# sonniki/image-captioning-with-external-knowledge

Hardware: AMD Instinct MI355X
Metric: decode_steps_per_sec (higher is better)
Workload: dtype f32 (3xbf16 split products, fp32 accumulate); 1 GPU; cfg2: geo variant, per-GPU batch 64 x 20 decode positions, 14x14x2048 features, K=20 knowledge rows, vocab 10000; global_batch=64, graph=True, collective_backend=none, split_allreduce=False, parallelism=dp1 (one flat-bucket all-reduce per step)

## Files before the change

### image-captioning-with-external-knowledge_amd/csrc/attention.hip

```cpp
#include <cstdlib>

#include "attention_mfma.h"
#include "common.h"

namespace ick {
namespace {

template <int DHP, bool VEC>
__global__ __launch_bounds__(256) void attn_kernel(ick_attn_args p, int TQ, int SLD) {
    chain_priority();
    constexpr int VLD = DHP + 4;
    constexpr int G = DHP / 4;
    extern __shared__ __attribute__((aligned(16))) float smem[];
    const int S = p.S, dh = p.dh;
    float* Vs = smem;
    float* Qs = Vs + S * VLD;
    float* Ps = Qs + TQ * DHP;
    float* rowinv = Ps + TQ * SLD;

    const int h = blockIdx.x, b = blockIdx.y, t0 = blockIdx.z * TQ;
    const int nt = min(TQ, p.T - t0);
    const int tid = threadIdx.x, lane = tid & 63, wave = tid >> 6;
    const Dropout drop = make_dropout(p.drop_p, epoch_seed(p.drop_seed, p.drop_epoch), p.drop_site);
    int slen = S;
// ... 318 lines not shown
    if (dir == 0) {
        pl.tq = attn_fwd_chunk(T, S, DHP);
        if (attn_fwd_floats(pl.tq, S, DHP) > kAttnBudget) return ICK_EINVAL;
    } else {
        pl.tq = attn_bwd_chunk(T, S, DHP);
        if (attn_bwd_floats(pl.tq, S, DHP) > kAttnBudget) return ICK_EINVAL;
    }
    pl.chunks = ceil_div(T, pl.tq);
    pl.overwrites = dir == 0 || pl.chunks == 1;
    return 0;
}

}
}

extern "C" int ick_attention(const ick_attn_args* in, void* stream) {
    using namespace ick;
    if (!in) return ICK_EINVAL;
    const ick_attn_args& a = *in;
    ICK_CHECK_ARG(a.Q && a.K && a.V && a.O);
    ICK_CHECK_ARG(a.B > 0 && a.H > 0 && a.T > 0 && a.S > 0 && a.dh > 0 && a.dh <= 64);
    ICK_CHECK_ARG(a.B <= 65535);
    hipStream_t s = (hipStream_t)stream;
    AttnPlan pl;
    if (int e = attn_plan(0, a.T, a.S, a.dh, attn_head_major(a, a.dh <= 32 ? 32 : 64), pl)) return e;
    if (pl.mfma) return launch_attn_mfma(a, s);
    if (pl.dhp == 32) return launch_attn<32>(a, pl.tq, s);
    return launch_attn<64>(a, pl.tq, s);
}


extern "C" int ick_attention_bwd(const ick_attn_bwd_args* in, void* stream) {
    using namespace ick;
    if (!in) return ICK_EINVAL;
    const ick_attn_bwd_args& a = *in;
    ICK_CHECK_ARG(a.Q && a.K && a.V && a.O && a.dO && a.lse && a.dQ && a.dK && a.dV);
    ICK_CHECK_ARG(a.B > 0 && a.B <= 65535 && a.H > 0 && a.T > 0 && a.S > 0 && a.dh > 0 && a.dh <= 64);
    const int DHP = a.dh <= 32 ? 32 : 64;
    ICK_CHECK_ARG(attn_head_major(a, DHP));
    hipStream_t s = (hipStream_t)stream;
    AttnPlan pl;
    if (int e = attn_plan(1, a.T, a.S, a.dh, true, pl)) return e;
    if (pl.mfma) return launch_attn_bwd_mfma(a, s);
    if (pl.dhp == 32) return launch_attn_bwd<32>(a, pl.tq, s);
    return launch_attn_bwd<64>(a, pl.tq, s);
}

extern "C" int ick_attention_bwd_overwrites(int32_t T, int32_t S, int32_t dh) {
    using namespace ick;
    AttnPlan pl;
    return attn_plan(1, T, S, dh, true, pl) == 0 && pl.overwrites ? 1 : 0;
}

extern "C" int ick_attention_plan(int32_t dir, int32_t T, int32_t S, int32_t dh, int32_t head_major, int32_t* out) {
    using namespace ick;
    if (!out) return ICK_EINVAL;
    AttnPlan pl;
    const int e = attn_plan(dir, T, S, dh, head_major != 0, pl);
    const int v[7] = {pl.mfma, pl.nqt, pl.maxt, pl.dhp, pl.tq, pl.chunks, pl.overwrites};
    for (int i = 0; i < 7; ++i) out[i] = v[i];
    return e;
}
```

### image-captioning-with-external-knowledge_amd/csrc/attention_mfma.h

```cpp
#pragma once
#include "common.h"

namespace ick {

constexpr int kAttnMfmaUnsupported = -1000;

bool attn_mfma_shape_ok(int T, int S, int dh);
int attn_mfma_nqt(int T);
int attn_mfma_maxt(int S);
template <class Args>
inline bool attn_head_major(const Args& a, int DHP) {
    auto al16 = [](const void* q) { return (reinterpret_cast<uintptr_t>(q) & 15) == 0; };
    return a.q_ts == DHP && a.k_ss == DHP && a.v_ss == DHP && al16(a.Q) && al16(a.K) && al16(a.V) && a.q_bs % 4 == 0 &&
           a.q_hs % 4 == 0 && a.k_bs % 4 == 0 && a.k_hs % 4 == 0 && a.v_bs % 4 == 0 && a.v_hs % 4 == 0;
}
int launch_attn_mfma(const ick_attn_args& a, hipStream_t s);
int launch_attn_bwd_mfma(const ick_attn_bwd_args& a, hipStream_t s);

}
```

### image-captioning-with-external-knowledge_amd/csrc/attention_mfma.hip

```cpp
#include <algorithm>

#include "attention_mfma.h"

#ifdef ICK_ATTN_STAMPS
__device__ unsigned long long ick_attn_stamps[4][16];
#define ICK_ASTAMP(kern, i)                                                                   \
    do {                                                                                      \
        if (threadIdx.x == 0 && blockIdx.x == 0 && blockIdx.y == 0) ick_attn_stamps[kern][i] = __builtin_readcyclecounter(); \
    } while (0)
extern "C" int ick_debug_read_attn_stamps(unsigned long long* out) {
    return (int)hipMemcpyFromSymbol(out, HIP_SYMBOL(ick_attn_stamps), sizeof(ick_attn_stamps));
}
#else
#define ICK_ASTAMP(kern, i)
#endif

namespace ick {
namespace {

constexpr int DHP = 32;
constexpr int QLD = DHP + 4;

__device__ __forceinline__ float4 mask_cols(float4 x, int c0, int dh) {
    x.x = c0 + 0 < dh ? x.x : 0.f; x.y = c0 + 1 < dh ? x.y : 0.f;
    x.z = c0 + 2 < dh ? x.z : 0.f; x.w = c0 + 3 < dh ? x.w : 0.f;
    return x;
}

__device__ __forceinline__ int wave_id_of(unsigned tid) { return __builtin_amdgcn_readfirstlane((int)(tid >> 6)); }

__device__ __forceinline__ f32x4 mfma4(const float4& a, const float4& b, f32x4 c) {
    c = __builtin_amdgcn_mfma_f32_16x16x4f32(a.x, b.x, c, 0, 0, 0);
    c = __builtin_amdgcn_mfma_f32_16x16x4f32(a.y, b.y, c, 0, 0, 0);
    c = __builtin_amdgcn_mfma_f32_16x16x4f32(a.z, b.z, c, 0, 0, 0);
    c = __builtin_amdgcn_mfma_f32_16x16x4f32(a.w, b.w, c, 0, 0, 0);
    return c;
}

template <int IT>
__device__ __forceinline__ void stage_transposed_load(const float* __restrict__ src, int rows, float4 (&x)[IT]) {
#pragma unroll
    for (int it = 0; it < IT; ++it) {
        const int f = threadIdx.x + 256 * it;
        const int s = f >> 3, c = f & 7;
        x[it] = *reinterpret_cast<const float4*>(src + (int64_t)(s < rows ? s : 0) * DHP + 4 * c);
    }
}
template <int IT>
__device__ __forceinline__ void stage_transposed_store(const float4 (&x)[IT], float* __restrict__ dst, int rows,
                                                       int rows_pad, int SP, int dh) {
#pragma unroll
    for (int it = 0; it < IT; ++it) {
        const int f = threadIdx.x + 256 * it;
        const int s = f >> 3, c = f & 7;
        if (s < rows_pad) {
            const float4 v = mask_cols(x[it], 4 * c, s < rows ? dh : 0);
            dst[(4 * c + 0) * SP + s] = v.x; dst[(4 * c + 1) * SP + s] = v.y;
            dst[(4 * c + 2) * SP + s] = v.z; dst[(4 * c + 3) * SP + s] = v.w;
// ... 116 lines not shown
        }
        s += __shfl_xor(s, 16, 64);
        s += __shfl_xor(s, 32, 64);
        sum[qt] = s;
    }
    f32x4 oacc[NQT][2];
#pragma unroll
    for (int qt = 0; qt < NQT; ++qt) {
#pragma unroll
        for (int jt = 0; jt < 2; ++jt) {
            f32x4 acc = {0.f, 0.f, 0.f, 0.f};
#pragma unroll
            for (int i = 0; i < MAXT; ++i) {
                if (wave + 4 * i < nkt) {
                    const float4 vt = *reinterpret_cast<const float4*>(Vt + (16 * jt + li) * SP + 16 * (wave + 4 * i) + 4 * lq);
                    const float4 pf = make_float4(sc[i][qt][0], sc[i][qt][1], sc[i][qt][2], sc[i][qt][3]);
                    acc = mfma4(vt, pf, acc);
                }
            }
            oacc[qt][jt] = acc;
        }
        if (lq == 0) rsum[wave * NQ + 16 * qt + li] = sum[qt];
    }
    ICK_ASTAMP(SK, 6);
    __syncthreads();
    ICK_ASTAMP(SK, 7);
#pragma unroll
    for (int qt = 0; qt < NQT; ++qt)
#pragma unroll
        for (int jt = 0; jt < 2; ++jt)
            *reinterpret_cast<f32x4*>(Ored + ((wave * NQT + qt) * 2 + jt) * 256 + lane * 4) = oacc[qt][jt];
    if (tid < NQ) {
        const float s = (rsum[tid] + rsum[NQ + tid]) + (rsum[2 * NQ + tid] + rsum[3 * NQ + tid]);
        stat[NQ + tid] = s > 0.f ? 1.f / s : 0.f;
        if (p.lse && tid < T) p.lse[((int64_t)b * p.H + h) * T + tid] = stat[tid] + __logf(s);
    }
    __syncthreads();
    for (int tt = wave; tt < NQT * 2; tt += 4) {
        const int qt = tt >> 1, jt = tt & 1;
        f32x4 o = {0.f, 0.f, 0.f, 0.f};
#pragma unroll
        for (int w = 0; w < 4; ++w) o += *reinterpret_cast<const f32x4*>(Ored + ((w * NQT + qt) * 2 + jt) * 256 + lane * 4);
        const int query = 16 * qt + li;
        if (query < T) {
            const float inv = stat[NQ + query];
            float* orow = p.O + (int64_t)b * p.o_bs + (int64_t)query * p.o_ts + h * dh;
            const int j0 = 16 * jt + 4 * lq;
#pragma unroll
            for (int r = 0; r < 4; ++r)
                if (j0 + r < dh) orow[j0 + r] = o[r] * inv;
        }
    }
    ICK_ASTAMP(SK, 8);
}

template <int NQT, int MAXT>
__global__ __launch_bounds__(256) void attn_bwd_mfma_kernel(ick_attn_bwd_args p, int SP, bool st2) {
    chain_priority_bwd();
    [[maybe_unused]] constexpr int SK = MAXT > 1 ? 3 : 2;
    ICK_ASTAMP(SK, 0);
    constexpr int NQ = NQT * 16;
    constexpr int TLD = NQ + 4;
    extern __shared__ __attribute__((aligned(16))) float smem[];
    const int TR = (p.T + 3) & ~3;
    float* dSs = smem;
    float* Qs = dSs + TR * SP;
    float* Gs = Qs + NQ * QLD;
    float* Qt = Gs + NQ * QLD;
    float* Gt = Qt + DHP * TLD;
    float* Ls = Gt + DHP * TLD;
    float* Dl = Ls + NQ;
    float* Kw = Dl + NQ + (wave_id_of(threadIdx.x)) * (16 * QLD);
    float* dQp = Qs;

    const int b = blockIdx.x, h = blockIdx.y;
    const int tid = threadIdx.x, lane = tid & 63, wave = tid >> 6;
    const int li = lane & 15, lq = lane >> 4;
    const int T = p.T, S = p.S, dh = p.dh;
    const int nkt = (S + 15) >> 4;
    const Dropout drop = make_dropout(p.drop_p, epoch_seed(p.drop_seed, p.drop_epoch), p.drop_site);
    const float* qb = p.Q + (int64_t)b * p.q_bs + (int64_t)h * p.q_hs;
    const float* kb = p.K + (int64_t)b * p.k_bs + (int64_t)h * p.k_hs;
    const float* vb = p.V + (int64_t)b * p.v_bs + (int64_t)h * p.v_hs;
    const float* ob = p.O + (int64_t)b * p.o_bs + h * dh;
    const float* gb = p.dO + (int64_t)b * p.o_bs + h * dh;

    constexpr int QIT = (NQ * 8 + 255) / 256;
    float4 qx[QIT];
#pragma unroll
    for (int it = 0; it < QIT; ++it) {
        const int f = tid + 256 * it;
        const int t = f >> 3, c = f & 7;
        qx[it] = *reinterpret_cast<const float4*>(qb + (int64_t)(t < T ? t : 0) * DHP + 4 * c);
    }
    const float lse_v = p.lse[((int64_t)b * p.H + h) * T + (tid < T ? tid : 0)];
    float gv[NQT * 2], ov[NQT * 2];
#pragma unroll
    for (int it = 0; it < NQT * 2; ++it) {
        const int f = tid + 256 * it;
        const int t = f >> 5, j = f & 31;
        const bool ok = t < T && j < dh;
        const int64_t at = ok ? (int64_t)t * p.o_ts + j : 0;
        gv[it] = gb[at];
        ov[it] = ob[at];
    }
    float4 kf[MAXT][2], vf[MAXT][2];
// ... 145 lines not shown
        const int qt = tt >> 1, jt = tt & 1;
        const int j = 16 * jt + li;
        f32x4 acc = {0.f, 0.f, 0.f, 0.f};
#pragma unroll
        for (int w = 0; w < 4; ++w) acc += *reinterpret_cast<const f32x4*>(dQp + ((w * NQT + qt) * 2 + jt) * 256 + lane * 4);
        if (j < dh) {
#pragma unroll
            for (int r = 0; r < 4; ++r) {
                const int query = 16 * qt + 4 * lq + r;
                if (query < T) p.dQ[(int64_t)b * p.dq_bs + (int64_t)query * p.dq_ts + h * dh + j] = acc[r];
            }
        }
    }
    ICK_ASTAMP(SK, 6);
}

template <int NQT, int MAXT>
int launch_fwd(const ick_attn_args& a, int SP, hipStream_t s) {
    const size_t fl = std::max<size_t>((size_t)DHP * SP, 4 * NQT * 2 * 256) + (size_t)NQT * 16 * QLD + 10 * NQT * 16;
    if (fl * sizeof(float) > 150 * 1024) return kAttnMfmaUnsupported;
    auto kern = attn_fwd_mfma_kernel<NQT, MAXT>;
    static LdsAttrOnce attr;
    if (int e = attr.ensure((const void*)kern, 160 * 1024)) return e;
    hipLaunchKernelGGL(kern, dim3(a.H, a.B), dim3(256), fl * sizeof(float), s, a, SP);
    ICK_LAUNCH_RET();
}

template <int NQT, int MAXT>
int launch_bwd(const ick_attn_bwd_args& a, int SP, hipStream_t s) {
    constexpr int NQ = NQT * 16;
    const size_t tr = (size_t)((a.T + 3) & ~3);
    const size_t fl = std::max(tr * SP + 2 * (size_t)NQ * QLD + 2 * (size_t)DHP * (NQ + 4) + 2 * NQ + 4 * 16 * QLD,
                               (size_t)NQ * SP + 64);
    if (fl * sizeof(float) > 150 * 1024) return kAttnMfmaUnsupported;
    auto kern = attn_bwd_mfma_kernel<NQT, MAXT>;
    static LdsAttrOnce attr;
    if (int e = attr.ensure((const void*)kern, 160 * 1024)) return e;
    const bool st2 = a.dh % 2 == 0 && a.dk_bs % 2 == 0 && a.dk_ss % 2 == 0 && a.dv_bs % 2 == 0 && a.dv_ss % 2 == 0 &&
                     (reinterpret_cast<uintptr_t>(a.dK) & 7) == 0 && (reinterpret_cast<uintptr_t>(a.dV) & 7) == 0;
    hipLaunchKernelGGL(kern, dim3(a.B, a.H), dim3(256), fl * sizeof(float), s, a, SP, st2);
    ICK_LAUNCH_RET();
}

}

bool attn_mfma_shape_ok(int T, int S, int dh) {
    if (!(T >= 2 && T <= 64 && S >= 1 && S <= 512 && dh <= DHP)) return false;
    const size_t nq = (size_t)((T + 15) / 16) * 16, sp = (size_t)((S + 15) / 16) * 16 + 4, tr = (size_t)((T + 3) & ~3);
    return std::max(tr * sp + 2 * nq * QLD + 2 * DHP * (nq + 4) + 2 * nq + 4 * 16 * QLD, nq * sp + 64) * sizeof(float) <= 150 * 1024;
}

int attn_mfma_nqt(int T) { return (T + 15) / 16; }

int attn_mfma_maxt(int S) { return S <= 64 ? 1 : (S <= 256 ? 4 : (S <= 320 ? 5 : 8)); }

int launch_attn_mfma(const ick_attn_args& a, hipStream_t s) {
    if (!attn_mfma_shape_ok(a.T, a.S, a.dh)) return kAttnMfmaUnsupported;
    if (!attn_head_major(a, DHP)) return kAttnMfmaUnsupported;
    const int SP = ((a.S + 15) / 16) * 16 + 4;
    const int nqt = attn_mfma_nqt(a.T);
    const int mt = attn_mfma_maxt(a.S);
#define ICK_FWD(N)                                                                                   \
    case N: return mt == 1 ? launch_fwd<N, 1>(a, SP, s) : (mt == 4 ? launch_fwd<N, 4>(a, SP, s) :   \
                   (mt == 5 ? launch_fwd<N, 5>(a, SP, s) : launch_fwd<N, 8>(a, SP, s)))
    switch (nqt) {
        ICK_FWD(1); ICK_FWD(2); ICK_FWD(3); ICK_FWD(4);
    }
#undef ICK_FWD
    return kAttnMfmaUnsupported;
}

int launch_attn_bwd_mfma(const ick_attn_bwd_args& a, hipStream_t s) {
    if (!attn_mfma_shape_ok(a.T, a.S, a.dh)) return kAttnMfmaUnsupported;
    const int SP = ((a.S + 15) / 16) * 16 + 4;
    const int mt = attn_mfma_maxt(a.S);
#define ICK_BWD(N)                                                                                   \
    case N: return mt == 1 ? launch_bwd<N, 1>(a, SP, s) : (mt == 4 ? launch_bwd<N, 4>(a, SP, s) :   \
                   (mt == 5 ? launch_bwd<N, 5>(a, SP, s) : launch_bwd<N, 8>(a, SP, s)))
    switch (attn_mfma_nqt(a.T)) {
        ICK_BWD(1); ICK_BWD(2); ICK_BWD(3); ICK_BWD(4);
    }
#undef ICK_BWD
    return kAttnMfmaUnsupported;
}

}
```

### image-captioning-with-external-knowledge_amd/lib.py

```python
import ctypes as C
import os

_PKG = os.path.dirname(os.path.abspath(__file__))
LIB_PATH = os.path.join(_PKG, "libick_amd.so")
if os.environ.get("ICK_LIB_PATH"):
    LIB_PATH = os.environ["ICK_LIB_PATH"]

ICK_GEO, ICK_KNOWLEDGE, ICK_NEWS = 0, 1, 2
VARIANT_ID = {"geo": ICK_GEO, "knowledge": ICK_KNOWLEDGE, "news": ICK_NEWS}
GEMM_RELU, GEMM_ACCUM, GEMM_ATOMIC, GEMM_COLSUM_ONLY = 1, 2, 4, 16

vp = C.c_void_p
i32 = C.c_int32
i64 = C.c_int64
f32 = C.c_float
u32 = C.c_uint32


class GemmArgs(C.Structure):
    _fields_ = [
        ("A", vp), ("B", vp), ("C", vp), ("bias", vp),
        ("M", i32), ("N", i32), ("K", i32),
        ("a_rs", i64), ("a_ks", i64), ("a_grp", i32), ("a_gs", i64), ("a_gmap", vp),
        ("b_rs", i64), ("b_ks", i64),
# ... 145 lines not shown
    "ick_gemm": [C.POINTER(GemmArgs), vp],
    "ick_gemm_plan": [C.POINTER(GemmArgs), C.POINTER(GemmPlanInfo)],
    "ick_set_gemm_split": [i32],
    "ick_get_gemm_split": [],
    "ick_presplit_bytes": [i32, i32, C.POINTER(i64)],
    "ick_presplit_weights": [C.POINTER(PresplitItem), i32, vp],
    "ick_rowchain_supported": [i32, i32, i32],
    "ick_rowchain_fwd": [C.POINTER(RowChainArgs), vp],
    "ick_rowchain_bwd_supported": [i32, i32, i32],
    "ick_rowchain_bwd": [C.POINTER(RowChainBwdArgs), vp],
    "ick_pack_weights": [C.POINTER(PackItem), i32, vp],
    "ick_packed_weight_floats": [i32, i32, C.POINTER(i64)],
    "ick_add_layernorm": [vp, vp, vp, vp, vp, i64, i32, f32, i64, i64, i64, vp, vp, f32, u32, u32, vp, vp],
    "ick_attention": [C.POINTER(AttnArgs), vp],
    "ick_entity_encode": [i32, vp, i32, vp, vp, i32, vp, i32, vp, i32, i32, i32, i32, vp],
    "ick_fact_encode": [vp, vp, vp, i32, vp, i32, i32, i32, i32, vp],
    "ick_caption_embed": [vp, vp, vp, vp, vp, vp, vp, vp, i32, i32, i32, i32, i32, i32, i32, f32, i32, f32, u32, u32,
                          vp, vp],
    "ick_context_indicators": [vp, vp, vp, vp, vp, vp, i32, i32, i32, i32, i32, i32, i32, i32, i32, vp],
    "ick_pointer_scores": [vp, vp, vp, vp, vp, vp, i32, i32, i32, i32, i64, i32, vp, vp],
    "ick_mul": [vp, vp, vp, i64, vp],
    "ick_dropout_mask": [vp, i64, i32, f32, u32, u32, vp],
    "ick_top2": [vp, i64, i32, i32, vp, vp, vp],
    "ick_greedy_update": [vp, vp, vp, vp, vp, vp, vp, i32, i32, i32, i32, i32, i32, i32, vp],
    "ick_greedy_select": [vp, i64, i32, i32, vp, vp, vp, vp, vp, i32, i32, i32, i32, i32, i32, vp],
    "ick_packed_ce": [vp, i64, vp, vp, i32, i32, i32, i32, vp, vp, vp, vp, vp],
    "ick_packed_ce_weighted": [vp, i64, vp, vp, vp, i32, i32, i32, i32, vp, vp, vp, vp, vp],
    "ick_samples_to_captions": [vp, i32, i32, i32, i32, i32, i32, i32, i32, vp, vp, vp, vp],
    "ick_cider_d": [vp, i32, i32, vp, i32, i32, i32, vp, vp, i32, f32, f32, i32, i32, i32, vp, i32, i32, vp, i32,
                    vp, vp, vp],
    "ick_decode_supported": [i32, i32, i32, i32, i32],
    "ick_decode_plan": [i32, i32, i32, i32, i32, C.POINTER(i32)],
    "ick_decode_layers": [C.POINTER(DecodeCtx), i32, vp],
    "ick_decode_layers_part": [C.POINTER(DecodeCtx), i32, i32, vp],
    "ick_decode_layers_attn": [C.POINTER(DecodeCtx), vp, i32, i32, vp],
    "ick_decode_init": [C.POINTER(DecodeCtx), i32, i32, vp],
    "ick_decode_select_greedy": [C.POINTER(DecodeCtx), i32, vp],
    "ick_decode_select_beam": [C.POINTER(DecodeCtx), C.POINTER(BeamState), i32, vp],
    "ick_decode_beam_supported": [i32, i32],
    "ick_decode_select_sample": [C.POINTER(DecodeCtx), C.POINTER(SampleState), i32, vp],
    "ick_decode_sample_supported": [i32, i32],
    "ick_decode_select_beam_rules": [C.POINTER(DecodeCtx), C.POINTER(BeamState), C.POINTER(DecodeRules), i32, vp],
    "ick_decode_select_sample_rules": [C.POINTER(DecodeCtx), C.POINTER(SampleState), C.POINTER(DecodeRules), i32, vp],
    "ick_decode_select_beam_diverse": [C.POINTER(DecodeCtx), C.POINTER(BeamState), C.POINTER(DecodeRules),
                                       C.POINTER(DecodeDiversity), i32, vp],
    "ick_decode_select_beam_forced": [C.POINTER(DecodeCtx), C.POINTER(BeamState), C.POINTER(DecodeRules),
                                      C.POINTER(DecodeConstraints), i32, vp],
    "ick_attention_bwd": [C.POINTER(AttnBwdArgs), vp],
    "ick_layernorm_bwd": [vp, vp, vp, vp, vp, vp, vp, vp, vp, i64, i32, vp, f32, u32, u32, vp, vp, vp],
    "ick_layernorm_bwd_rows_per_block": [],
    "ick_gemm_grouped": [vp, i32, vp],
    "ick_attention_bwd_overwrites": [i32, i32, i32],
    "ick_attention_plan": [i32, i32, i32, i32, i32, C.POINTER(i32)],
    "ick_relu_bwd": [vp, vp, vp, i64, f32, vp],
    "ick_colsum": [vp, i64, i32, i64, vp, vp],
    "ick_caption_embed_bwd": [vp, vp, vp, vp, vp, vp, i32, i32, i32, i32, i32, i32, i32, f32, f32, u32, u32, vp, vp],
    "ick_pointer_scores_bwd": [vp, i64, i32, vp, vp, vp, vp, vp, vp, vp, vp, i32, i32, i32, i32, vp],
    "ick_entity_encode_bwd": [i32, vp, vp, i32, vp, vp, i32, vp, i32, vp, i32, i32, i32, vp],
    "ick_fact_encode_bwd": [vp, vp, vp, vp, i32, i32, i32, i32, i32, vp],
    "ick_context_gate_bwd": [vp, vp, vp, vp, vp, i32, i32, i32, i32, i32, i32, i32, i32, i32, vp],
    "ick_adam_clamp": [vp, vp, vp, vp, i64, f32, f32, f32, f32, f32, f32, i32, vp, vp, vp],
    "ick_adam_clamp_derive": [vp, vp, vp, vp, vp, vp, i32, f32, f32, f32, f32, f32, f32, i32, vp, vp, vp],
    "ick_grad_sqnorm_plan": [i64, C.POINTER(i32)],
    "ick_grad_sqnorm": [vp, i64, f32, vp, vp, i64, vp, vp],
    "ick_adam_opt": [vp, vp, vp, vp, i64, f32, f32, vp, LrSchedule, f32, f32, f32, i32, vp, vp, vp],
    "ick_adam_opt_derive": [vp, vp, vp, vp, vp, vp, i32, f32, f32, vp, LrSchedule, f32, f32, f32, i32, vp, vp, vp],
    "ick_adam_ema": [vp, vp, vp, vp, vp, i64, f32, f32, f32, vp, LrSchedule, f32, f32, f32, i32, vp, vp, vp, i32, vp],
    "ick_adam_ema_derive": [vp, vp, vp, vp, vp, vp, vp, i32, f32, f32, f32, vp, LrSchedule, f32, f32, f32, i32, vp, vp, vp,
                            i32, vp],
    "ick_adam_decay": [vp, vp, vp, vp, vp, i64, f32, f32, f32, vp, LrSchedule, f32, f32, f32, i32, vp, vp, vp, i32, vp, vp,
                       i64, i32, vp],
    "ick_adam_decay_derive": [vp, vp, vp, vp, vp, vp, vp, i32, f32, f32, f32, vp, LrSchedule, f32, f32, f32, i32, vp, vp, vp,
                              i32, vp, vp, i64, i32, vp],
    "ick_conv1_wgrad_plan": [i32, i32, i32, i32, C.POINTER(i32), C.POINTER(i64)],
    "ick_conv1_wgrad": [vp, vp, vp, vp, i32, i32, i32, i32, vp, i64, vp],
    "ick_counter_add": [vp, u32, vp],
    "ick_counter_add_if": [vp, u32, vp, vp],
    "ick_timestamp": [vp, vp],
    "ick_copy_batch": [vp, vp, vp, i32, vp],
    "ick_scale_by_ratio": [vp, i64, vp, vp, vp],
    "ick_head_rowmap": [vp, i32, i32, vp, vp, vp, vp],
    "ick_pointer_scores_packed": [vp, vp, vp, vp, vp, vp, i32, i32, i32, i32, i64, i32, vp, vp, vp],
    "ick_packed_ce_packed": [vp, i64, vp, vp, vp, vp, i32, i32, i32, i32, vp, vp, vp, vp, vp],
    "ick_packed_ce_smooth": [vp, i64, vp, vp, vp, vp, vp, vp, i32, i32, i32, i32, vp, vp, vp, vp, vp],
    "ick_pointer_scores_bwd_packed": [vp, i64, i32, vp, vp, vp, vp, vp, vp, vp, vp, i32, i32, i32, i32, vp, vp, vp],
    "ick_gather_rows": [vp, i64, vp, vp, vp, i64, i32, i32, vp],
    "ick_row_logprob_rank": [vp, i64, vp, vp, vp, i32, i32, i32, i32, vp, vp, vp, vp],
    "ick_caption_score_sums": [vp, i32, i32, i32, vp, vp, vp, vp, vp, vp, vp, vp, vp, vp],
    "ick_sched_sample_mix": [vp, i64, vp, vp, vp, vp, i32, i32, i32, i32, i32, i32, i32, vp, vp, vp, vp, i32, vp, vp, vp,
                             vp],
    "ick_caption_metrics": [vp, i32, i32, vp, i32, i32, i32, i32, i32, i32, vp, i32, i32, C.c_double, i32, vp, i32, vp,
                            vp, vp, vp, vp, vp, vp, vp, vp],
    "ick_caption_metric_sums": [vp, vp, vp, i32, vp, vp, vp, vp],
    "ick_geo_reference_counts": [vp, i32, i32, vp, vp, vp, i32, i32, i32, i32, C.POINTER(i32), i32, i32, i32, vp, i32, vp,
                                 i32, i32, i64, i64, i64, vp, vp, vp, vp],
}

_lib = None
PROFILE = None
_proxy = None


class IckError(RuntimeError):
    pass


# ... 28 lines not shown
```

### image-captioning-with-external-knowledge_amd/ops.py

```python
import contextlib
import ctypes as C
import gc
import math
import os

import torch

from . import lib as L


def _p(t):
    return None if t is None else t.data_ptr()


def _stream():
    return torch.cuda.current_stream().cuda_stream


def _f32c(t, name):
    if t.dtype != torch.float32 or not t.is_cuda:
        raise L.IckError("%s must be a float32 device tensor (got %s on %s)" % (name, t.dtype, t.device))
    return t


# ... 901 lines not shown
    if N < 1 or not 1 <= T <= GEO_MAX_T:
        raise L.IckError("geo_reference_counts: N >= 1 and 1 <= T <= %d (got %d, %d)" % (GEO_MAX_T, N, T))
    if B < 1 or not 1 <= K <= GEO_MAX_K or Cf < 5:
        raise L.IckError("geo_reference_counts: entities need B >= 1, 1 <= K <= %d and C >= 5" % GEO_MAX_K)
    if tuple(entity_names.shape) != (B, K, 2 + GEO_NAME_CHARS):
        raise L.IckError("geo_reference_counts: entity_names must be (%d, %d, %d)" % (B, K, 2 + GEO_NAME_CHARS))
    for t, name in ((bins_distance, "bins_distance"), (bins_azimuth, "bins_azimuth")):
        if t.shape[1] != 2 or not 1 <= t.shape[0] <= GEO_MAX_BINS:
            raise L.IckError("geo_reference_counts: %s holds 1..%d [lo, hi] rows" % (name, GEO_MAX_BINS))
    if isinstance(n_types, bool) or not isinstance(n_types, int) or not 1 <= n_types <= GEO_MAX_TYPES:
        raise L.IckError("geo_reference_counts: 1 <= n_types <= %d" % GEO_MAX_TYPES)
    trigger_ids = [int(i) for i in trigger_ids]
    ids = trigger_ids + [int(of_id), int(the_id), int(a_id)]
    if len(trigger_ids) != GEO_TERMS or not isinstance(V, int) or V < 1 or not all(-1 <= i < V for i in ids):
        raise L.IckError("geo_reference_counts: 8 trigger ids and the ids of of / the / a, each -1 or in [0, V)")
    if not isinstance(image_index, torch.Tensor) or image_index.shape != (N,):
        raise L.IckError("geo_reference_counts needs an (N,) image_index")
    if not 0 <= int(row_offset) <= 2 ** 62 or not -2 ** 63 <= int(seed) < 2 ** 64:
        raise L.IckError("geo_reference_counts: row_offset >= 0 and a 64-bit seed")
    dev = tokens.device
    idx = image_index.to(device=dev, dtype=torch.int32).contiguous()
    seed = int(seed) & (2 ** 64 - 1)
    seed -= 2 ** 64 if seed >= 2 ** 63 else 0
    ld = 1 + 2 * GEO_MAX_BINS + (n_types + 63) // 64 * 64
    hist = torch.zeros(2, GEO_TERMS, ld, device=dev, dtype=torch.int32)
    marks = torch.empty(N, T, device=dev, dtype=torch.int32)
    trig = (C.c_int32 * GEO_TERMS)(*trigger_ids)
    L.check(L.load().ick_geo_reference_counts(_p(tokens), N, T, _p(idx), _p(entities), _p(entity_names), B, K, Cf, V, trig,
                                              int(of_id), int(the_id), int(a_id), _p(bins_distance),
                                              bins_distance.shape[0], _p(bins_azimuth), bins_azimuth.shape[0], n_types,
                                              ld, seed, int(row_offset), _p(marks), _p(hist[0]), _p(hist[1]), _stream()),
            "ick_geo_reference_counts")
    return hist[0], hist[1], marks


def attention_bwd_buffer(shape, T, S, dh, device):
    if L.load().ick_attention_bwd_overwrites(T, S, dh):
        return torch.empty(shape, device=device, dtype=torch.float32)
    return torch.zeros(shape, device=device, dtype=torch.float32)


ATTN_PLAN_KEYS = ("mfma", "nqt", "maxt", "dhp", "tq", "chunks", "overwrites")


def attention_plan(direction, T, S, dh, head_major=True):
    out = (C.c_int32 * len(ATTN_PLAN_KEYS))()
    rc = L.load_raw().ick_attention_plan({"fwd": 0, "bwd": 1}[direction], T, S, dh, int(head_major), out)
    if rc == -1:
        return None
    L.check(rc, "ick_attention_plan")
    return dict(zip(ATTN_PLAN_KEYS, (int(v) for v in out)))


def attention_heads_bwd(q, kv, O, dO, lse, dQ, dK, dV, H, dh, T, S, q_seg=0, k_seg=0, v_seg=1, causal=False,
                        drop=None, q_pos0=0):
    B = q.shape[0]
    Tq, Sa = q.shape[3], kv.shape[3]
    hp = q.shape[4]
    assert kv.shape[4] == hp
    a = L.AttnBwdArgs()
    a.Q = q.data_ptr() + 4 * (q_seg * H * Tq * hp)
    a.K = kv.data_ptr() + 4 * (k_seg * H * Sa * hp)
    a.V = kv.data_ptr() + 4 * (v_seg * H * Sa * hp)
    a.O, a.dO, a.lse = _p(O), _p(dO), _p(lse)
    a.dQ, a.dK, a.dV = _p(dQ), _p(dK), _p(dV)
    a.B, a.H, a.T, a.S, a.dh = B, H, T, S, dh
    a.q_bs, a.q_hs, a.q_ts = q.stride(0), Tq * hp, hp
    a.k_bs, a.k_hs, a.k_ss = kv.stride(0), Sa * hp, hp
    a.v_bs, a.v_hs, a.v_ss = kv.stride(0), Sa * hp, hp
    a.o_bs, a.o_ts = O.stride(0), O.stride(1)
    a.dq_bs, a.dq_ts = dQ.stride(0), dQ.stride(1)
    a.dk_bs, a.dk_ss = dK.stride(0), dK.stride(1)
    a.dv_bs, a.dv_ss = dV.stride(0), dV.stride(1)
    a.scale = 1.0 / math.sqrt(dh)
    a.causal, a.q_pos0 = int(causal), q_pos0
    _drop(a, drop)
    L.check(L.load().ick_attention_bwd(C.byref(a), _stream()), "ick_attention_bwd")


def layernorm_bwd(dy, x, res, gamma, mean, rstd, dgamma, dbeta, drop=None):
    d = x.shape[-1]
    rows = x.numel() // d
    dz = torch.empty_like(x)
    dxd = torch.empty_like(x)
    rpb = L.load().ick_layernorm_bwd_rows_per_block()
    part = torch.empty((rows + rpb - 1) // rpb, 2 * d, device=x.device, dtype=torch.float32)
    L.check(L.load().ick_layernorm_bwd(_p(dy), _p(x), _p(res), _p(gamma), _p(mean), _p(rstd), _p(dz), None, None,
                                       rows, d, _p(dxd), *_dargs(drop), _p(part), _stream()), "ick_layernorm_bwd")

    if SIDE is not None:
        SIDE.flush()
    ln_partials_reduce(part, dgamma, dbeta)
    return dz, dxd


def ln_partials_reduce(part, dgamma, dbeta):
    d = part.shape[1] // 2
    adjacent = dbeta.data_ptr() == dgamma.data_ptr() + 4 * d
    if SIDE is not None:
        if adjacent:
            SIDE.add_problem(colsum_problem(part, dgamma), part)
        else:
            SIDE.add_problem(colsum_problem(part[:, :d], dgamma), part)
            SIDE.add_problem(colsum_problem(part[:, d:], dbeta), part)
    elif adjacent:
        colsum(part, dgamma, n_out=2 * d)
# ... 404 lines not shown
```

### include/ick_amd.h

```cpp
#ifndef ICK_AMD_H
#define ICK_AMD_H

#include <stdint.h>

#ifdef __cplusplus
extern "C" {
#endif

#define ICK_OK 0
#define ICK_EINVAL (-1)
#define ICK_EALIGN (-2)
#define ICK_EWORKSPACE (-3)

#define ICK_MAX_LAYERS 8

int ick_version(void);
int ick_set_deterministic(int on);
int ick_get_deterministic(void);
int ick_device_info(int* num_cu, int* wave_size, char* arch_name, int arch_name_len);

typedef struct {
    const float* A; const float* B; float* C; const float* bias;
    int32_t M, N, K;
    int64_t a_rs, a_ks; int32_t a_grp; int64_t a_gs; const int32_t* a_gmap;
// ... 225 lines not shown
} ick_decode_diversity;
int ick_decode_select_beam_diverse(const ick_decode_ctx* ctx, const ick_beam_state* beam,
                                   const ick_decode_rules* rules ,
                                   const ick_decode_diversity* div, int32_t pos, void* stream);

typedef struct {
    const int32_t* force;
    int32_t* met;
} ick_decode_constraints;
int ick_decode_select_beam_forced(const ick_decode_ctx* ctx, const ick_beam_state* beam,
                                  const ick_decode_rules* rules ,
                                  const ick_decode_constraints* constraints, int32_t pos, void* stream);

int ick_packed_ce(const float* scores, int64_t ld, const int64_t* captions_sorted, const int32_t* decode_len,
                  int32_t B, int32_t L, int32_t Vx, int32_t pad_token, float* row_loss ,
                  float* loss_sum, float* count, float* dscores, void* stream);
int ick_packed_ce_weighted(const float* scores, int64_t ld, const int64_t* captions_sorted, const int32_t* decode_len,
                           const float* weights, int32_t B, int32_t L, int32_t Vx, int32_t pad_token,
                           float* row_loss , float* loss_sum, float* count, float* dscores,
                           void* stream);
int ick_samples_to_captions(const int64_t* tokens, int32_t R, int32_t T, int32_t V, int32_t K, int32_t has_facts,
                            int32_t start_token, int32_t end_token, int32_t pad_token, int64_t* captions, int64_t* masks,
                            int64_t* lengths, void* stream);

int ick_cider_d(const int64_t* cand, int32_t N, int32_t T, const int64_t* refs, int32_t B, int32_t M, int32_t Lr,
                const uint32_t* df_keys, const int32_t* df_count, int32_t U, float log_ref_len, float sigma,
                int32_t start_token, int32_t end_token, int32_t pad_token, const int32_t* ignore, int32_t n_ignore,
                int32_t mode, const int32_t* image_index, int32_t num_samples, float* rewards, float* advantages,
                void* stream);

int ick_caption_metrics(const int64_t* cand, int32_t N, int32_t T, const int64_t* refs, int32_t B, int32_t M, int32_t Lr,
                        int32_t start_token, int32_t end_token, int32_t pad_token, const int32_t* ignore,
                        int32_t n_ignore, int32_t pointer_base, double beta, int32_t mode, const int32_t* image_index,
                        int32_t num_samples, const float* base_rewards, const float* weights, int32_t* counts,
                        float* bleu, float* rouge_l, int32_t* pointers, float* rewards, float* advantages, void* stream);

int ick_caption_metric_sums(const int32_t* counts, const float* rouge_l, const int32_t* pointers, int32_t N,
                            int64_t* sums, double* rouge_sum, int64_t* captions, void* stream);


typedef struct {
    const float* Q; const float* K; const float* V; const float* O; const float* dO; const float* lse;
    float* dQ; float* dK; float* dV;
    int32_t B, H, T, S, dh;
    int64_t q_bs, q_hs, q_ts, k_bs, k_hs, k_ss, v_bs, v_hs, v_ss, o_bs, o_ts;
    int64_t dq_bs, dq_ts, dk_bs, dk_ss, dv_bs, dv_ss;
    float scale; int32_t causal; int32_t q_pos0;
    float drop_p; uint32_t drop_seed, drop_site;
    const uint32_t* drop_epoch;
} ick_attn_bwd_args;
int ick_attention_bwd(const ick_attn_bwd_args* args, void* stream);
int ick_attention_bwd_overwrites(int32_t T, int32_t S, int32_t dh);
int ick_attention_plan(int32_t dir, int32_t T, int32_t S, int32_t dh, int32_t head_major, int32_t* out);

int ick_layernorm_bwd_rows_per_block(void);
int ick_layernorm_bwd(const float* dy, const float* x, const float* res, const float* gamma, const float* mean,
                      const float* rstd, float* dz, float* dgamma, float* dbeta, int64_t rows, int32_t d,
                      float* dx_drop ,
                      float drop_p, uint32_t drop_seed, uint32_t drop_site, const uint32_t* drop_epoch, float* partials,
                      void* stream);
int ick_relu_bwd(const float* dy, const float* act, float* dx, int64_t n, float scale ,
                 void* stream);
int ick_colsum(const float* a, int64_t M, int32_t N, int64_t ld, float* out, void* stream);
int ick_caption_embed_bwd(const float* dx, const int64_t* captions, const int64_t* masks, float* dword,
                          float* dee, float* dfe, int32_t B, int32_t L, int32_t K, int32_t F, int32_t V,
                          int32_t d, int32_t pad_token, float scale, float drop_p, uint32_t drop_seed,
                          uint32_t drop_site, const uint32_t* drop_epoch, void* stream);
int ick_pointer_scores_bwd(const float* ds, int64_t ds_ld, int32_t col0, const float* h, const float* ctx,
                           const float* w, const float* ind, float* dh, float* dctx, float* dw, float* dbias,
                           int32_t B, int32_t T, int32_t Kc, int32_t d, void* stream);
int ick_entity_encode_bwd(int32_t variant, const float* dee, const float* entities, int32_t ent_cols,
                          const float* ee, const float* word_emb, int32_t vocab, float* dtype_emb,
                          int32_t ntypes, float* dword, int32_t B, int32_t K, int32_t d, void* stream);
int ick_fact_encode_bwd(const float* dfe, const int64_t* facts, float* dee, float* dpred, int32_t num_pred,
                        int32_t B, int32_t K, int32_t F, int32_t d, void* stream);
int ick_context_gate_bwd(const int64_t* captions, const int64_t* facts, const float* dgate, float* dw,
                         float* dbias, int32_t B, int32_t L, int32_t T, int32_t K, int32_t F, int32_t V,
                         int32_t num_pred, int32_t d, int32_t mode, void* stream);
int ick_adam_clamp(float* p, float* g, float* m, float* v, int64_t n, float gscale, float clip, float lr,
                   float beta1, float beta2, float eps, int32_t step, const uint32_t* step_ptr,
                   const float* gscale_den, void* stream);
typedef struct ick_adam_item {
    int64_t off;
    int32_t rows, K, drow0, Nd;
    float* pack;
    float* pack_t;
    float* copy;
    void* ps;
    void* ps_t;
    float* tr;
    int64_t copy_ld, tr_ld;
} ick_adam_item;
typedef struct ick_adam_block {
    int32_t item, tn, tk, cnt4;
    int64_t off4;
    float* copy;
} ick_adam_block;
int ick_adam_clamp_derive(float* p, float* g, float* m, float* v, const ick_adam_item* items,
                          const ick_adam_block* blocks, int32_t n_blocks, float gscale, float clip, float lr,
                          float beta1, float beta2, float eps, int32_t step, const uint32_t* step_ptr,
                          const float* gscale_den, void* stream);

#define ICK_OPT_WORDS 8
enum { ICK_LR_CONSTANT = 0, ICK_LR_INVERSE_SQRT = 1, ICK_LR_COSINE = 2, ICK_LR_LINEAR = 3 };
typedef struct ick_lr_schedule {
    int32_t kind, warmup, total;
// ... 91 lines not shown
```

Before: 820,500 decode-steps/s.

## Add per-wave MFMA forward attention kernel for short sequences

Adds a forward attention kernel in which each wavefront independently handles one (batch, head, 16-query tile), holding Q/K in registers and staging V transposed in a per-wave LDS slice, using only wave-level barriers. It is selected when T and S are at most 32, replacing the block-wide kernel that needs block barriers and a cross-wave reduction. The aim is to cut synchronisation and launch granularity for the small decoder attention shapes. An env var can disable it, and a query helper is exposed to Python.

```diff
diff --git a/image-captioning-with-external-knowledge_amd/csrc/attention.hip b/image-captioning-with-external-knowledge_amd/csrc/attention.hip
--- a/image-captioning-with-external-knowledge_amd/csrc/attention.hip
+++ b/image-captioning-with-external-knowledge_amd/csrc/attention.hip
@@ -394,6 +394,12 @@
     return attn_plan(1, T, S, dh, true, pl) == 0 && pl.overwrites ? 1 : 0;
 }
 
+extern "C" int ick_attention_wave_form(int32_t dir, int32_t T, int32_t S, int32_t dh, int32_t head_major) {
+    using namespace ick;
+    AttnPlan pl;
+    return attn_plan(dir, T, S, dh, head_major != 0, pl) == 0 && pl.mfma && attn_mfma_wave_form(dir, T, S, dh) ? 1 : 0;
+}
+
 extern "C" int ick_attention_plan(int32_t dir, int32_t T, int32_t S, int32_t dh, int32_t head_major, int32_t* out) {
     using namespace ick;
     if (!out) return ICK_EINVAL;
diff --git a/image-captioning-with-external-knowledge_amd/csrc/attention_mfma.h b/image-captioning-with-external-knowledge_amd/csrc/attention_mfma.h
--- a/image-captioning-with-external-knowledge_amd/csrc/attention_mfma.h
+++ b/image-captioning-with-external-knowledge_amd/csrc/attention_mfma.h
@@ -8,6 +8,7 @@
 bool attn_mfma_shape_ok(int T, int S, int dh);
 int attn_mfma_nqt(int T);
 int attn_mfma_maxt(int S);
+bool attn_mfma_wave_form(int dir, int T, int S, int dh);
 template <class Args>
 inline bool attn_head_major(const Args& a, int DHP) {
     auto al16 = [](const void* q) { return (reinterpret_cast<uintptr_t>(q) & 15) == 0; };
diff --git a/image-captioning-with-external-knowledge_amd/csrc/attention_mfma.hip b/image-captioning-with-external-knowledge_amd/csrc/attention_mfma.hip
--- a/image-captioning-with-external-knowledge_amd/csrc/attention_mfma.hip
+++ b/image-captioning-with-external-knowledge_amd/csrc/attention_mfma.hip
@@ -3,7 +3,7 @@
 #include "attention_mfma.h"
 
 #ifdef ICK_ATTN_STAMPS
-__device__ unsigned long long ick_attn_stamps[4][16];
+__device__ unsigned long long ick_attn_stamps[5][16];
 #define ICK_ASTAMP(kern, i)                                                                   \
     do {                                                                                      \
         if (threadIdx.x == 0 && blockIdx.x == 0 && blockIdx.y == 0) ick_attn_stamps[kern][i] = __builtin_readcyclecounter(); \
@@ -226,6 +226,142 @@
         }
     }
     ICK_ASTAMP(SK, 8);
+}
+
+template <int NQT, int NKT>
+__global__ __launch_bounds__(256) void attn_fwd_wave_kernel(ick_attn_args p, int nwaves) {
+    chain_priority();
+    ICK_ASTAMP(4, 0);
+    constexpr int VLD = 16 * NKT + 4;
+    __shared__ __attribute__((aligned(16))) float lds[4][DHP * VLD];
+    const int lane = threadIdx.x & 63, li = lane & 15, lq = lane >> 4;
+    const int wave = wave_id_of(threadIdx.x);
+    const int w = blockIdx.x * 4 + wave;
+    if (w >= nwaves) return;
+    float* Vt = lds[wave];
+    const int unit = w / NQT, qt = w - unit * NQT;
+    const int b = unit / p.H, h = unit - b * p.H;
+    const int T = p.T, S = p.S, dh = p.dh;
+    int slen = S;
+    if (p.kv_len) slen = __builtin_amdgcn_readfirstlane(min(S, p.kv_len[b]));
+    const float* qb = p.Q + (int64_t)b * p.q_bs + (int64_t)h * p.q_hs;
+    const float* kb = p.K + (int64_t)b * p.k_bs + (int64_t)h * p.k_hs;
+    const float* vb = p.V + (int64_t)b * p.v_bs + (int64_t)h * p.v_hs;
+    const int query = 16 * qt + li;
+
+    float4 qf[2], kf[NKT][2], vx[2 * NKT];
+    {
+        const float* qr = qb + (int64_t)(query < T ? query : 0) * DHP + 4 * lq;
+#pragma unroll
+        for (int t = 0; t < 2; ++t) qf[t] = *reinterpret_cast<const float4*>(qr + 16 * t);
+    }
+#pragma unroll
+    for (int kt = 0; kt < NKT; ++kt) {
+        const float* kr = kb + (int64_t)(16 * kt + li < slen ? 16 * kt + li : 0) * DHP + 4 * lq;
+#pragma unroll
+        for (int t = 0; t < 2; ++t) kf[kt][t] = *reinterpret_cast<const float4*>(kr + 16 * t);
+    }
+#pragma unroll
+    for (int it = 0; it < 2 * NKT; ++it) {
+        const int key = (lane >> 3) + 8 * it;
+        vx[it] = *reinterpret_cast<const float4*>(vb + (int64_t)(key < slen ? key : 0) * DHP + 4 * (lane & 7));
+    }
+    const Dropout drop = make_dropout(p.drop_p, epoch_seed(p.drop_seed, p.drop_epoch), p.drop_site);
+#pragma unroll
+    for (int t = 0; t < 2; ++t) qf[t] = mask_cols(qf[t], 16 * t + 4 * lq, query < T ? dh : 0);
+#pragma unroll
+    for (int kt = 0; kt < NKT; ++kt)
+#pragma unroll
+        for (int t = 0; t < 2; ++t) kf[kt][t] = mask_cols(kf[kt][t], 16 * t + 4 * lq, 16 * kt + li < slen ? dh : 0);
+    ICK_ASTAMP(4, 1);
+
+    bool live[NKT];
+#pragma unroll
+    for (int kt = 0; kt < NKT; ++kt) live[kt] = 16 * kt < slen && !(p.causal && 16 * kt > p.q_pos0 + 16 * qt + 15);
+
+    f32x4 sc[NKT];
+    float m = -INFINITY;
+#pragma unroll
+    for (int kt = 0; kt < NKT; ++kt) {
+        f32x4 acc = {0.f, 0.f, 0.f, 0.f};
+        if (live[kt]) {
+            acc = mfma4(kf[kt][0], qf[0], acc);
+            acc = mfma4(kf[kt][1], qf[1], acc);
+        }
+#pragma unroll
+        for (int r = 0; r < 4; ++r) {
+            const int key = 16 * kt + 4 * lq + r;
+            float v = acc[r] * p.scale;
+            if (key >= slen || (p.causal && key > p.q_pos0 + query)) v = -INFINITY;
+            acc[r] = v;
+            m = fmaxf(m, v);
+        }
+        sc[kt] = acc;
+    }
+#pragma unroll
+    for (int it = 0; it < 2 * NKT; ++it) {
+        const int key = (lane >> 3) + 8 * it, c = lane & 7;
+        const float4 v = mask_cols(vx[it], 4 * c, key < slen ? dh : 0);
+        Vt[(4 * c + 0) * VLD + key] = v.x; Vt[(4 * c + 1) * VLD + key] = v.y;
+        Vt[(4 * c + 2) * VLD + key] = v.z; Vt[(4 * c + 3) * VLD + key] = v.w;
+    }
+    m = fmaxf(m, __shfl_xor(m, 16, 64));
+    m = fmaxf(m, __shfl_xor(m, 32, 64));
+    const uint32_t rowbase = (uint32_t)((b * p.H + h) * T + query) * (uint32_t)S;
+    float s = 0.f;
+#pragma unroll
+    for (int kt = 0; kt < NKT; ++kt) {
+        float st = 0.f;
+#pragma unroll
+        for (int r = 0; r < 4; ++r) {
+            const int key = 16 * kt + 4 * lq + r;
+            const float e = (m == -INFINITY) ? 0.f : __expf(sc[kt][r] - m);
+            st += e;
+            sc[kt][r] = drop.on() ? e * drop.mask(rowbase + (uint32_t)key) : e;
+        }
+        st += __shfl_xor(st, 16, 64);
+        st += __shfl_xor(st, 32, 64);
+        s += st;
+    }
+    const float inv = s > 0.f ? 1.f / s : 0.f;
+    if (p.lse && lq == 0 && query < T) p.lse[((int64_t)b * p.H + h) * T + query] = m + __logf(s);
+    ICK_ASTAMP(4, 2);
+
+    __builtin_amdgcn_fence(__ATOMIC_RELEASE, "wavefront");
+    __builtin_amdgcn_wave_barrier();
+    float* orow = p.O + (int64_t)b * p.o_bs + (int64_t)query * p.o_ts + h * dh;
+#pragma unroll
+    for (int jt = 0; jt < 2; ++jt) {
+        f32x4 o = {0.f, 0.f, 0.f, 0.f};
+#pragma unroll
+        for (int kt = 0; kt < NKT; ++kt)
+            if (live[kt]) {
+                const float4 vt = *reinterpret_cast<const float4*>(Vt + (16 * jt + li) * VLD + 16 * kt + 4 * lq);
+                o += mfma4(vt, make_float4(sc[kt][0], sc[kt][1], sc[kt][2], sc[kt][3]), f32x4{0.f, 0.f, 0.f, 0.f});
+            }
+        const int j0 = 16 * jt + 4 * lq;
+        if (query < T) {
+#pragma unroll
+            for (int r = 0; r < 4; ++r)
+                if (j0 + r < dh) orow[j0 + r] = o[r] * inv;
+        }
+    }
+    ICK_ASTAMP(4, 3);
+}
+
+bool attn_no_wave() {
+    static const bool v = getenv("ICK_ATTN_NO_WAVE") != nullptr;
+    return v;
+}
+
+template <int NQT>
+int launch_fwd_wave(const ick_attn_args& a, hipStream_t s) {
+    const int nwaves = a.B * a.H * NQT;
+    if (a.S <= 16)
+        hipLaunchKernelGGL((attn_fwd_wave_kernel<NQT, 1>), dim3((nwaves + 3) / 4), dim3(256), 0, s, a, nwaves);
+    else
+        hipLaunchKernelGGL((attn_fwd_wave_kernel<NQT, 2>), dim3((nwaves + 3) / 4), dim3(256), 0, s, a, nwaves);
+    ICK_LAUNCH_RET();
 }
 
 template <int NQT, int MAXT>
@@ -477,6 +613,10 @@
 
 int attn_mfma_nqt(int T) { return (T + 15) / 16; }
 
+bool attn_mfma_wave_form(int dir, int T, int S, int dh) {
+    return dir == 0 && !attn_no_wave() && attn_mfma_shape_ok(T, S, dh) && T <= 32 && S <= 32;
+}
+
 int attn_mfma_maxt(int S) { return S <= 64 ? 1 : (S <= 256 ? 4 : (S <= 320 ? 5 : 8)); }
 
 int launch_attn_mfma(const ick_attn_args& a, hipStream_t s) {
@@ -484,6 +624,7 @@
     if (!attn_head_major(a, DHP)) return kAttnMfmaUnsupported;
     const int SP = ((a.S + 15) / 16) * 16 + 4;
     const int nqt = attn_mfma_nqt(a.T);
+    if (attn_mfma_wave_form(0, a.T, a.S, a.dh)) return nqt == 1 ? launch_fwd_wave<1>(a, s) : launch_fwd_wave<2>(a, s);
     const int mt = attn_mfma_maxt(a.S);
 #define ICK_FWD(N)                                                                                   \
     case N: return mt == 1 ? launch_fwd<N, 1>(a, SP, s) : (mt == 4 ? launch_fwd<N, 4>(a, SP, s) :   \
diff --git a/image-captioning-with-external-knowledge_amd/lib.py b/image-captioning-with-external-knowledge_amd/lib.py
--- a/image-captioning-with-external-knowledge_amd/lib.py
+++ b/image-captioning-with-external-knowledge_amd/lib.py
@@ -221,6 +221,7 @@
     "ick_gemm_grouped": [vp, i32, vp],
     "ick_attention_bwd_overwrites": [i32, i32, i32],
     "ick_attention_plan": [i32, i32, i32, i32, i32, C.POINTER(i32)],
+    "ick_attention_wave_form": [i32, i32, i32, i32, i32],
     "ick_relu_bwd": [vp, vp, vp, i64, f32, vp],
     "ick_colsum": [vp, i64, i32, i64, vp, vp],
     "ick_caption_embed_bwd": [vp, vp, vp, vp, vp, vp, i32, i32, i32, i32, i32, i32, i32, f32, f32, u32, u32, vp, vp],
diff --git a/image-captioning-with-external-knowledge_amd/ops.py b/image-captioning-with-external-knowledge_amd/ops.py
--- a/image-captioning-with-external-knowledge_amd/ops.py
+++ b/image-captioning-with-external-knowledge_amd/ops.py
@@ -977,6 +977,10 @@
     return dict(zip(ATTN_PLAN_KEYS, (int(v) for v in out)))
 
 
+def attention_wave_form(direction, T, S, dh, head_major=True):
+    return int(L.load_raw().ick_attention_wave_form({"fwd": 0, "bwd": 1}[direction], T, S, dh, int(head_major)))
+
+
 def attention_heads_bwd(q, kv, O, dO, lse, dQ, dK, dV, H, dh, T, S, q_seg=0, k_seg=0, v_seg=1, causal=False,
                         drop=None, q_pos0=0):
     B = q.shape[0]
diff --git a/include/ick_amd.h b/include/ick_amd.h
--- a/include/ick_amd.h
+++ b/include/ick_amd.h
@@ -301,6 +301,7 @@
 int ick_attention_bwd(const ick_attn_bwd_args* args, void* stream);
 int ick_attention_bwd_overwrites(int32_t T, int32_t S, int32_t dh);
 int ick_attention_plan(int32_t dir, int32_t T, int32_t S, int32_t dh, int32_t head_major, int32_t* out);
+int ick_attention_wave_form(int32_t dir, int32_t T, int32_t S, int32_t dh, int32_t head_major);
 
 int ick_layernorm_bwd_rows_per_block(void);
 int ick_layernorm_bwd(const float* dy, const float* x, const float* res, const float* gamma, const float* mean,
```

New measurement: 819,600 decode-steps/s. No clear change (-0.1%).
